# janinethoma/soft_contrastive_learning

Measured on AMD Instinct MI355X. Metric: train-step images/sec (VGG16-NetVLAD soft-MS, 640x480), higher is better.
Workload: dtype bf16; 1 GPU; configs[1]: wms soft-contrastive train step, VGG16-NetVLAD K=64, 24 images/GPU 640x480, bf16 backbone, float32-accurate NetVLAD + f32 loss; global_batch=24, locations=1200, parallelism=dp1, optimizer=adam

## Files before the change

### soft_contrastive_learning_amd/csrc/convh.hip

```cpp
#include <mutex>

#include "conv_lds.h"
#include "conv_pack_layout.h"

namespace {

constexpr int HBW = 40;
constexpr int HWC = HBW + 2;
constexpr int HPIX = 32;
constexpr int HCCH = 32;
constexpr int HNB = 128;
constexpr int HTPB = 3;
constexpr int HWT = 4 * HNB * 8;
constexpr int HTHR = 512;
constexpr int HX = 1;

template <int BHv>
struct HCfg {
  static constexpr int BH = BHv == 24 ? 12 : BHv;
  static constexpr int WR = BH + 2;
  static constexpr int SLOTS = WR * HWC * 4;
  static constexpr int NI = (SLOTS + 511) / 512;
  static constexpr int NA = (NI + 1) / 2;
  static constexpr int WIN = NI * 8 * 512;
  static constexpr int NMT = BH / 2 * 5;
  static constexpr int MT = BHv == 24 ? 15 : BH == 12 ? 8 : BH == 8 ? 10 : 4;
  static constexpr int NT = (BHv == 24 || BH == 8) ? 2 : 4;
  static constexpr int SPT = BHv == 24 ? 3 : 2;
  static constexpr int MH = MT / SPT;
  static constexpr size_t LDS = (2 * (size_t)WIN + 3 * HTPB * (size_t)HWT) * 2;
};

template <int V>
struct HConst {
  static constexpr int value = V;
};

__device__ __forceinline__ int ht_row(int i) { return (i >= 4 && i < 12) ? 1 : 0; }
__device__ __forceinline__ int ht_col(int i) { return i < 4 ? i : i < 8 ? i - 4 : i < 12 ? i - 4 : i - 8; }

__global__ __launch_bounds__(256) void convh_pack_kernel(const void* __restrict__ w, int64_t sk,
                                                         int64_t sc, int64_t sh, int64_t sw,
                                                         int flags, int cin, int kout,
                                                         unsigned short* __restrict__ packed) {
  const int transposed = flags & 1, wf32 = flags & 2;
  const int64_t idx = (int64_t)blockIdx.x * 256 + threadIdx.x;
  const int64_t total = (int64_t)9 * (cin / HCCH) * kout * HCCH;
  if (idx >= total) return;
  const int64_t off = pack_src_offset(pack_lds_coord(idx, cin), sk, sc, sh, sw, transposed);
  packed[idx] = weight_bf16(w, off, wf32);
}

template <int EPI, int BHv, bool STAMP = false, bool FULL = false>
__global__ __launch_bounds__(HTHR, 1) void convh_kernel(const unsigned short* __restrict__ x,
                                                       const unsigned short* __restrict__ packed,
                                                       int B, int H, int W, int cin, int kout,
                                                       unsigned short* __restrict__ out,
                                                       const float* __restrict__ bias, int relu,
                                                       const unsigned short* __restrict__ mask,
                                                       unsigned char* __restrict__ pidx,
                                                       int vblocks) {
  using G = HCfg<BHv>;
  constexpr int BH = G::BH, WR = G::WR, WIN = G::WIN, NMT = G::NMT, MT = G::MT, NT = G::NT;
  constexpr int MH = G::MH, NI = G::NI, NA = G::NA, SPT = G::SPT;
  constexpr bool WEAVE = BHv == 24 || BHv == 6 || BHv == 8;
  constexpr int HS = 9 * SPT;
  extern __shared__ __attribute__((aligned(16))) unsigned short lds[];
  unsigned short* win = lds;
  unsigned short* wts = lds + 2 * WIN;
  const int lane = threadIdx.x & 63;
  const int wid = __builtin_amdgcn_readfirstlane(threadIdx.x >> 6);
  const int i = lane & 15, g = lane >> 4;
  const int kb = kout / HNB;
  const int blocks_x = (W + HBW - 1) / HBW, blocks_y = (H + BH - 1) / BH;
  const int CC = cin / HCCH, S = 9 * CC;
  const unsigned short* zeros = reinterpret_cast<const unsigned short*>(zero_block);
  int nb = 0, b = 0, y0 = 0, x0 = 0;
  int rel[NI];
#pragma unroll
  for (int n = 0; n < NI; ++n) {
    const int slot = 64 * (wid + 8 * n) + lane;
    const int pix = slot >> 2, row = pix / HWC, col = pix - row * HWC;
    const int piece = (slot & 3) ^ (((col >> 2) & 1) | ((row & 1) << 1));
    rel[n] = pix >= WR * HWC ? -1 : (row << 16) | (col << 8) | piece;
  }
  int woff[NI];
  auto locate = [&](int vb) -> bool {
    const int grp = vb / (8 * kb), rem = vb - grp * 8 * kb;
    const int pblk = grp * 8 + (rem & 7);
    nb = rem >> 3;
    if (pblk >= B * blocks_x * blocks_y) return false;
    b = pblk / (blocks_x * blocks_y);
    const int t2 = pblk % (blocks_x * blocks_y);
    y0 = (t2 / blocks_x) * BH;
    x0 = (t2 % blocks_x) * HBW;
#pragma unroll
    for (int n = 0; n < NI; ++n) {
      int r = rel[n];
      asm volatile("" : "+v"(r));
      const int y = y0 - 1 + (r >> 16), xx = x0 - 1 + ((r >> 8) & 255);
      const bool inimg = r >= 0 && y >= 0 && y < H && xx >= 0 && xx < W;
      woff[n] = inimg ? ((b * H + y) * W + xx) * cin + 8 * (r & 255) : -1;
    }
    return true;
  };
  auto issue_win = [&](int cc, int buf, int n0, int n1) {
    const unsigned base = lds_byte_of(win) + buf * WIN * 2;
#pragma unroll
    for (int n = 0; n < NI; ++n)
      if (n >= n0 && n < n1)
        glds16(woff[n] >= 0 ? x + woff[n] + HCCH * cc : zeros, base + (wid + 8 * n) * 1024);
  };
  auto issue_wts = [&](int grp, int buf) {
    const unsigned short* src = packed + ((int64_t)nb * S + HTPB * grp) * HWT + lane * 8;
    const unsigned base = lds_byte_of(wts) + buf * HTPB * HWT * 2;
#pragma unroll
    for (int n = 0; n < 3; ++n) {
      const int j = wid + 8 * n;
      glds16(src + j * 512, base + j * 1024);
    }
  };
  auto issue_wts_one = [&](int grp, int buf, int n) {
    const unsigned short* src = packed + ((int64_t)nb * S + HTPB * grp) * HWT + lane * 8;
    const unsigned base = lds_byte_of(wts) + buf * HTPB * HWT * 2;
    const int j = wid + 8 * n;
    glds16(src + j * 512, base + j * 1024);
  };
  auto stage_first = [&]() {
    issue_wts(0, 0);
    issue_wts(1, 1);
    issue_win(0, 0, 0, NI);
  };
  const int mg = NT == 4 ? wid >> 1 : wid >> 2, ng = NT == 4 ? wid & 1 : wid & 3;
  constexpr bool REG = MT % 5 == 0;
  constexpr bool ALLT = NMT % MT == 0;
  int aoff[MT];
#pragma unroll
  for (int j = 0; j < MT; ++j) {
    const int mt = MT * mg + j < NMT ? MT * mg + j : NMT - 1;
    aoff[j] = ((2 * (mt / 5)) * HWC + 8 * (mt % 5)) * HPIX;
  }
  const int lane_a = (ht_row(i) * HWC + ht_col(i)) * HPIX + (REG ? 2 * (MT / 5) * mg * HWC * HPIX : 0);
  int pieces = 0;
#pragma unroll
  for (int t = 0; t < 9; ++t) {
    const int r = ht_row(i) + t / 3, c = ht_col(i) + t % 3;
    pieces |= (g ^ (((c >> 2) & 1) | ((r & 1) << 1))) << (2 * t);
  }
  const int lane_b = (g * HNB + 16 * NT * ng + i) * 8;

  const int relu_in = relu;
  const int dbg = STAMP ? 0 : SCL_DIAG_ONLY(relu >> 1);
  relu &= 1;
  const short relu_floor = relu ? (short)0 : (short)-32768;
  bool staged = false;
  if (!STAMP && (dbg & 4) && wid >= 4) __builtin_amdgcn_s_setprio(1);
  uint64_t stamp[STAMP ? 24 : 1];
  int tcount = 0;
#define HSTAMP(k)                                                                     \
  if (STAMP)                                                                          \
  asm volatile("s_memtime %0\n\ts_waitcnt lgkmcnt(0)" : "=s"(stamp[STAMP ? (k) : 0])::"memory")
  for (int vb = blockIdx.x; vb < vblocks; vb += gridDim.x) {
    HSTAMP(0);
    if (!staged) {
      if (!locate(vb)) continue;
      stage_first();
    }
    staged = false;
    const int nb_t = nb, b_t = b, y0_t = y0, x0_t = x0;

    f32x4 acc[MT][NT];
#pragma unroll
    for (int j = 0; j < MT; ++j)
#pragma unroll
      for (int n = 0; n < NT; ++n) acc[j][n] = f32x4{0.f, 0.f, 0.f, 0.f};

    u32x4 af[2][MH], bf[2][NT];
    int tb = 0;
    auto load_half = [&](const unsigned short* wbase, int h, int par, int apar) {
      const int t = h / SPT, mh = h % SPT;
      if (mh == 0) {
        const unsigned short* wbp = wts + t * HWT + lane_b;
#pragma unroll
        for (int n = 0; n < NT; ++n)
          bf[(t + par) & 1][n] = *reinterpret_cast<const u32x4*>(wbp + 16 * n * 8);
        int pk = pieces;
        asm volatile("" : "+v"(pk));
        tb = lane_a + ((pk >> (2 * t)) & 3) * 8;
      }
#pragma unroll
      for (int j = 0; j < MH; ++j)
        af[(h + apar) & 1][j] = *reinterpret_cast<const u32x4*>(
            wbase + tb +
            (REG ? (2 * ((MH * mh + j) / 5) * HWC + 8 * ((MH * mh + j) % 5)) * HPIX : aoff[MH * mh + j]) +
            ((t / 3) * HWC + t % 3) * HPIX);
    };
    const int NG = 3 * CC;
    auto chunk = [&](int cc, auto par_c) {
      constexpr int PAR = decltype(par_c)::value;
      constexpr int APAR = PAR * (HS & 1);
      const unsigned short* wcur = win + (cc & 1) * WIN;
      const unsigned short* wnext = win + ((cc + 1) & 1) * WIN;
      const int ccn = cc + 1 < CC ? cc + 1 : cc;
      auto issue_op = [&](int gi, int k) {
        if (k < 3) {
          const int gn = 3 * cc + gi + 2 < NG ? 3 * cc + gi + 2 : NG - 3 + (gi + 2) % 3;
          issue_wts_one(gn, (gi + 2) % 3, k);
        } else {
          const int n = (gi == 0 ? 0 : NA) + k - 3;
          if (gi == 0 && n < NA) issue_win(ccn, (cc + 1) & 1, n, n + 1);
          if (gi == 1 && n < NI) issue_win(ccn, (cc + 1) & 1, n, n + 1);
        }
      };
#pragma unroll
      for (int h = 0; h < HS; ++h) {
        if (h + 1 < HS)
          load_half(wcur, h + 1, PAR, APAR);
        else
          load_half(wnext, 0, PAR ^ 1, APAR ^ (HS & 1));
        __builtin_amdgcn_sched_barrier(0);
        const int t = h / SPT, mh = h % SPT;
        const bool after_barrier = WEAVE && (h % (3 * SPT) == HX + 1);
#pragma unroll
        for (int j = 0; j < MH; ++j) {
#pragma unroll
          for (int n = 0; n < NT; ++n)
            acc[MH * mh + j][n] =
                EPI == 3 ? mfma16b(af[(h + APAR) & 1][j], bf[(t + PAR) & 1][n], acc[MH * mh + j][n])
                         : mfma16b(bf[(t + PAR) & 1][n], af[(h + APAR) & 1][j], acc[MH * mh + j][n]);
          if (after_barrier) {
            __builtin_amdgcn_sched_barrier(0);
#pragma unroll
            for (int k = j * 6 / MH; k < (j + 1) * 6 / MH; ++k) issue_op(h / (3 * SPT), k);
            __builtin_amdgcn_sched_barrier(0);
          }
        }
        if (h % (3 * SPT) == HX) {
          __builtin_amdgcn_sched_barrier(0);
          const int gi = h / (3 * SPT);
          if (gi == 1)
            asm volatile("s_waitcnt vmcnt(%0)" ::"n"(NA) : "memory");
          else
            asm volatile("s_waitcnt vmcnt(0)" ::: "memory");
          HSTAMP(2 + 9 * PAR + 3 * gi);
          __builtin_amdgcn_s_barrier();
          HSTAMP(2 + 9 * PAR + 3 * gi + 1);
          if (!WEAVE) {
            const int gn = 3 * cc + gi + 2 < NG ? 3 * cc + gi + 2 : NG - 3 + (gi + 2) % 3;
            issue_wts(gn, (gi + 2) % 3);
            if (gi == 0) issue_win(ccn, (cc + 1) & 1, 0, NA);
            if (gi == 1) issue_win(ccn, (cc + 1) & 1, NA, NI);
          }
          HSTAMP(2 + 9 * PAR + 3 * gi + 2);
        }
      }
    };

    if (!(dbg & 1)) {
      asm volatile("s_waitcnt vmcnt(0)" ::: "memory");
      __syncthreads();
    }
    HSTAMP(1);
    load_half(win, 0, 0, 0);
#pragma unroll 1
    for (int cc = 0; cc < CC; cc += 2) {
      chunk(cc, HConst<0>());
      chunk(cc + 1, HConst<1>());
    }

    int nb_e = nb_t, b_e = b_t, y0_e = y0_t, x0_e = x0_t;
    asm volatile("" : "+s"(nb_e), "+s"(b_e), "+s"(y0_e), "+s"(x0_e));
    HSTAMP(20);
    __builtin_amdgcn_s_barrier();
    HSTAMP(21);
    constexpr int SLD = 16 * NT + 8;
    constexpr int PCS = 2 * NT;
    constexpr int RR = 16 * PCS / 64;
    constexpr int SCRW = 16 * SLD + 8 * (16 * NT + 16);
    static_assert(4 * SCRW <= WIN && 4 * SCRW <= HTPB * HWT, "epilogue scratch must fit");
    unsigned short* scr = wid < 4 ? lds + WIN + wid * SCRW : wts + 2 * HTPB * HWT + (wid - 4) * SCRW;
    const int ch_w = HNB * nb_e + 16 * NT * ng;
    f32x4 bias4[EPI == 1 ? NT : 1];
    float bias1[EPI == 3 ? NT : 1];
    if (EPI == 1) {
#pragma unroll
      for (int n = 0; n < NT; ++n)
        bias4[n] = *reinterpret_cast<const f32x4*>(bias + ch_w + 16 * n + 4 * g);
    }
    if (EPI == 3) {
#pragma unroll
      for (int n = 0; n < NT; ++n) bias1[n] = bias[ch_w + 16 * n + i];
    }
    int piece_o[RR], piece_px[RR];
#pragma unroll
    for (int rr = 0; rr < RR; ++rr) {
      const int pp = lane + 64 * rr;
      piece_px[rr] = pp / PCS;
      piece_o[rr] = (ht_row(pp / PCS) * W + ht_col(pp / PCS)) * kout + 8 * (pp % PCS);
    }
    constexpr int PD = MT / 2;
    u32x4 mk[EPI == 2 ? MT : 1][EPI == 2 ? RR : 1];
    const int64_t tile_off = (((int64_t)b_e * H + y0_e) * W + x0_e) * kout + ch_w;
    const bool full_tile = FULL ? !(dbg & 2) : (y0_e + BH <= H && x0_e + HBW <= W && !(dbg & 2));
    auto load_mask = [&](int j) {
      const int mt = MT * mg + j;
      const int oy = y0_e + 2 * (mt / 5), ox = x0_e + 8 * (mt % 5);
      const unsigned short* mb = mask + tile_off + ((2 * (mt / 5)) * W + 8 * (mt % 5)) * kout;
#pragma unroll
      for (int rr = 0; rr < RR; ++rr) {
        if (FULL ? (ALLT || mt < NMT) : (full_tile && mt < NMT)) {
          mk[EPI == 2 ? j : 0][EPI == 2 ? rr : 0] = *reinterpret_cast<const u32x4*>(mb + piece_o[rr]);
        } else if (FULL) {
          mk[EPI == 2 ? j : 0][EPI == 2 ? rr : 0] = u32x4{0u, 0u, 0u, 0u};
        } else {
          const bool inside = mt < NMT && oy + ht_row(piece_px[rr]) < H && ox + ht_col(piece_px[rr]) < W;
          mk[EPI == 2 ? j : 0][EPI == 2 ? rr : 0] =
              inside ? *reinterpret_cast<const u32x4*>(mb + piece_o[rr]) : u32x4{0u, 0u, 0u, 0u};
        }
      }
    };
    if (EPI == 2) {
#pragma unroll
      for (int j = 0; j < PD; ++j) load_mask(j);
    }

    auto stage_next = [&]() {
      const int vn = vb + gridDim.x;
      if (vn < vblocks && locate(vn)) {
        asm volatile("s_waitcnt vmcnt(0)" ::: "memory");
        stage_first();
        staged = true;
      }
    };
    if (EPI != 2) stage_next();

    if (EPI == 3) {
      const int PH = H / 2, PW = W / 2;
      const bool upper = g == 0 || g == 3;
      const int cb = g < 2 ? 0 : 4;
      unsigned char* scr8 = reinterpret_cast<unsigned char*>(scr + 16 * SLD);
      constexpr int SLD8 = 16 * NT + 16;
#pragma unroll
      for (int jb = 0; jb < MT; jb += 4) {
#pragma unroll
        for (int jj = 0; jj < 4; ++jj) {
          const int j = jb + jj < MT ? jb + jj : MT - 1;
#pragma unroll
          for (int n = 0; n < NT; ++n) {
#pragma unroll
            for (int q0 = 0; q0 < 4; q0 += 2) {
              const float v0 = acc[j][n][q0], v1 = acc[j][n][q0 + 1];
              const float lm = fmaxf(v0, v1);
              const int li = v0 >= v1 ? 0 : 1;
              const float om = __shfl_xor(lm, 16);
              const int oi = __shfl_xor(li, 16);
              const float mu = upper ? lm : om, ml = upper ? om : lm;
              const int iu = upper ? li : oi, il = upper ? oi : li;
              const float m = fmaxf(mu, ml);
              const int k = mu >= ml ? iu : 2 + il;
              const int pl = 4 * jj + ((cb + q0) >> 1);
              if (upper) {
                scr[pl * SLD + 16 * n + i] = f32_to_bf16(fmaxf(m + bias1[n], 0.f));
                scr8[pl * SLD8 + 16 * n + i] = (unsigned char)k;
              }
            }
          }
        }
        __builtin_amdgcn_wave_barrier();
#pragma unroll
        for (int rr = 0; rr < RR; ++rr) {
          const int pp = lane + 64 * rr, pl = pp / PCS, pc = pp % PCS;
          const int mt = MT * mg + jb + (pl >> 2);
          const int py = (y0_e >> 1) + mt / 5, px = (x0_e >> 1) + 4 * (mt % 5) + (pl & 3);
          const u32x4 v = *reinterpret_cast<const u32x4*>(scr + pl * SLD + 8 * pc);
          if (jb + (pl >> 2) < MT && (FULL ? (ALLT || mt < NMT) : (mt < NMT && py < PH && px < PW && !(dbg & 2))))
            *reinterpret_cast<u32x4*>(out + (((int64_t)b_e * PH + py) * PW + px) * kout + ch_w + 8 * pc) = v;
        }
        if (lane < 16 * NT) {
          const int pl = lane / NT, pc = lane % NT;
          const int mt = MT * mg + jb + (pl >> 2);
          const int py = (y0_e >> 1) + mt / 5, px = (x0_e >> 1) + 4 * (mt % 5) + (pl & 3);
          const u32x4 v = *reinterpret_cast<const u32x4*>(scr8 + pl * SLD8 + 16 * pc);
          if (jb + (pl >> 2) < MT && (FULL ? (ALLT || mt < NMT) : (mt < NMT && py < PH && px < PW && !(dbg & 2))))
            *reinterpret_cast<u32x4*>(pidx + (((int64_t)b_e * PH + py) * PW + px) * kout + ch_w + 16 * pc) = v;
        }
        __builtin_amdgcn_wave_barrier();
      }
    } else {
      unsigned short* out_tile = out + tile_off;
#pragma unroll
      for (int j = 0; j < MT; ++j) {
        const int mt = MT * mg + j;
        if (ALLT || mt < NMT) {
          const int oy = y0_e + 2 * (mt / 5), ox = x0_e + 8 * (mt % 5);
          unsigned short* ob = out_tile + ((2 * (mt / 5)) * W + 8 * (mt % 5)) * kout;
#pragma unroll
          for (int n = 0; n < NT; ++n) {
            f32x4 v = acc[j][n];
            if (EPI == 1) v += bias4[n];
            unsigned p0 = pack2_bf16(v[0], v[1]), p1 = pack2_bf16(v[2], v[3]);
            if (EPI == 1) {
              p0 = max2_i16(p0, relu_floor);
              p1 = max2_i16(p1, relu_floor);
            }
            const u32x2 pk = {p0, p1};
            *reinterpret_cast<u32x2*>(scr + i * SLD + 16 * n + 4 * g) = pk;
          }
          __builtin_amdgcn_wave_barrier();
#pragma unroll
          for (int rr = 0; rr < RR; ++rr) {
            u32x4 v = *reinterpret_cast<const u32x4*>(scr + piece_px[rr] * SLD + 8 * ((lane + 64 * rr) % PCS));
            if (EPI == 2) v = relu_mask(v, mk[EPI == 2 ? j : 0][EPI == 2 ? rr : 0]);
            if (full_tile) {
              *reinterpret_cast<u32x4*>(ob + piece_o[rr]) = v;
            } else if (!FULL) {
              const bool inside = oy + ht_row(piece_px[rr]) < H && ox + ht_col(piece_px[rr]) < W && !(dbg & 2);
              if (inside) *reinterpret_cast<u32x4*>(ob + piece_o[rr]) = v;
            }
          }
          __builtin_amdgcn_wave_barrier();
        }
        if (EPI == 2) {
          __builtin_amdgcn_sched_barrier(0);
          if (j + PD < MT) load_mask(j + PD);
          if (j + PD == MT - 1) stage_next();
          __builtin_amdgcn_sched_barrier(0);
        }
      }
    }
    if (STAMP) {
      HSTAMP(22);
      if (threadIdx.x == 64 * ((relu_in >> 4) & 7) && (tcount == 1 || tcount == 2)) {
        uint64_t* o = reinterpret_cast<uint64_t*>(out + (int64_t)B * H * W * kout) +
                      (int64_t)(blockIdx.x * 2 + tcount - 1) * 24;
#pragma unroll
        for (int k = 0; k < 23; ++k) o[k] = stamp[STAMP ? k : 0];
      }
      ++tcount;
    }
  }
#undef HSTAMP
}

}

struct HGeom {
  const unsigned short* packed;
  int bh;
  LdsConvGrid grid;
};

template <int E, int BHV, bool STAMP = false, bool FULL = false>
static void convh_run(const LdsConvCall& c, const HGeom& g, int relu) {
  if constexpr (!STAMP && !FULL)
    if (c.H % HCfg<BHV>::BH == 0 && c.W % HBW == 0) return convh_run<E, BHV, false, true>(c, g, relu);
  static SclDeviceOnce once;
  scl_call_once(once, [] {
    (void)hipFuncSetAttribute(reinterpret_cast<const void*>(&convh_kernel<E, BHV, STAMP, FULL>),
                              hipFuncAttributeMaxDynamicSharedMemorySize, (int)HCfg<BHV>::LDS);
  });
  SCL_LAUNCH("convh_kernel", (convh_kernel<E, BHV, STAMP, FULL>), dim3(g.grid.gsize), dim3(HTHR),
             HCfg<BHV>::LDS, c.stream, (const unsigned short*)c.x, g.packed, c.B, c.H, c.W, c.cin,
             c.kout, (unsigned short*)c.out, c.bias, relu, (const unsigned short*)c.mask,
             (unsigned char*)c.pidx, g.grid.vblocks);
}
template <int BHV>
static void convh_epilogue(const LdsConvCall& c, const HGeom& g, int dbgbits) {
  if (c.pidx) convh_run<3, BHV>(c, g, dbgbits);
  else if (c.mask) convh_run<2, BHV>(c, g, dbgbits);
  else if (c.bias) convh_run<1, BHV>(c, g, (c.relu ? 1 : 0) | dbgbits);
  else convh_run<0, BHV>(c, g, 0);
}

#ifdef SCL_DIAG
static bool convh_diag(const LdsConvCall& c, const HGeom& g, int* rc);
#endif

int convh_launch(const LdsConvCall& c) {
  const int dv = SCL_DIAG_ONLY(c.dv);
  HGeom g;
  g.packed = (const unsigned short*)c.workspace;
  if (c.flags & SCL_W_PACKED) {
    g.packed = (const unsigned short*)c.w;
  } else {
    const int64_t total = (int64_t)9 * (c.cin / HCCH) * c.kout * HCCH;
    SCL_LAUNCH("convh_pack_kernel", convh_pack_kernel, dim3((unsigned)((total + 255) / 256)),
               dim3(256), 0, c.stream, c.w, c.sk, c.sc, c.sh, c.sw, c.flags, c.cin, c.kout,
               (unsigned short*)c.workspace);
  }
  const int bx = (c.W + HBW - 1) / HBW, kb = c.kout / HNB;
  const int cus = scl_conv_cus();
  g.bh = 12;
  int64_t best = -1;
  for (int cand : {12, 8, 6}) {
    const int64_t wg = (int64_t)c.B * ((c.H + cand - 1) / cand) * bx * kb;
    const int64_t cost = ((wg + cus - 1) / cus) * (cand + 2);
    if (best < 0 || cost < best) {
      best = cost;
      g.bh = cand;
    }
  }
  if (dv == 3012 || dv == 3008 || dv == 3006) g.bh = dv - 3000;
  if (dv == 3013) g.bh = 12;
  g.grid = lds_conv_grid((int64_t)c.B * ((c.H + g.bh - 1) / g.bh) * bx, kb, cus, dv);
#ifdef SCL_DIAG
  {
    int rc;
    if (convh_diag(c, g, &rc)) return rc;
  }
#endif
  const int dbgbits = (dv >= 3020 && dv < 3024) ? (dv - 3020) << 1 : (dv == 3040 ? 4 << 1 : 0);
  if (g.bh == 12) convh_epilogue<24>(c, g, dbgbits);
  else if (g.bh == 8) convh_epilogue<8>(c, g, dbgbits);
  else convh_epilogue<6>(c, g, dbgbits);
  return scl_launch_status();
}
```

### soft_contrastive_learning_amd/csrc/scl_common.h

```cpp
#pragma once
#include <hip/hip_runtime.h>
#include <stdint.h>
#include <stdlib.h>
#include <atomic>
#include <mutex>
#include <type_traits>

#include "scl_hip.h"
#include "scl_cdna4.h"

#define SCL_WAVE 64

__device__ __forceinline__ f32x16 zero16() {
  f32x16 z;
#pragma unroll
  for (int i = 0; i < 16; ++i) z[i] = 0.f;
  return z;
}

__device__ __forceinline__ float bf16_to_f32(unsigned short v) {
  return __uint_as_float(((unsigned)v) << 16);
}
__device__ __forceinline__ unsigned short f32_to_bf16(float f) {
  __bf16 b = (__bf16)f;
  return __builtin_bit_cast(unsigned short, b);
}

__device__ __forceinline__ unsigned pack2_bf16(float a, float b) {
  typedef __bf16 bf16x2_t __attribute__((ext_vector_type(2)));
  typedef float f32x2_t __attribute__((ext_vector_type(2)));
  const f32x2_t v = {a, b};
  return __builtin_bit_cast(unsigned, __builtin_convertvector(v, bf16x2_t));
}

__device__ __forceinline__ unsigned max2_i16(unsigned w, short floor16) {
  typedef short s16x2_t __attribute__((ext_vector_type(2)));
  const s16x2_t a = __builtin_bit_cast(s16x2_t, w), z = {floor16, floor16};
  return __builtin_bit_cast(unsigned, __builtin_elementwise_max(a, z));
}

__device__ __forceinline__ unsigned short weight_bf16(const void* w, int64_t i, int f32) {
  return f32 ? f32_to_bf16(static_cast<const float*>(w)[i])
             : static_cast<const unsigned short*>(w)[i];
}
__device__ __forceinline__ void store_weight_grad(void* gw, int64_t i, float v, int f32) {
  if (f32)
    static_cast<float*>(gw)[i] = v;
  else
    static_cast<unsigned short*>(gw)[i] = f32_to_bf16(v);
}

__device__ __forceinline__ unsigned relu_mask_word(unsigned g, unsigned y) {
  unsigned keep, out;
  asm("v_pk_max_i16 %0, %1, 0" : "=v"(keep) : "v"(y));
  asm("v_pk_min_i16 %0, %1, 1 op_sel_hi:[1,0]" : "=v"(keep) : "v"(keep));
  asm("v_pk_mul_lo_u16 %0, %1, %2" : "=v"(out) : "v"(g), "v"(keep));
  return out;
}
template <typename V4>
__device__ __forceinline__ V4 relu_mask(V4 g, V4 y) {
  return V4{relu_mask_word(g.x, y.x), relu_mask_word(g.y, y.y), relu_mask_word(g.z, y.z),
               relu_mask_word(g.w, y.w)};
}

template <typename T>
struct Elem;
template <>
struct Elem<float> {
  static __device__ __forceinline__ float ld(const float* p) { return *p; }
  static __device__ __forceinline__ f32x4 ld4(const float* p) {
    return *reinterpret_cast<const f32x4*>(p);
  }
  static __device__ __forceinline__ f32x2 ld2(const float* p) {
    return *reinterpret_cast<const f32x2*>(p);
  }
  static __device__ __forceinline__ void st(float* p, float v) { *p = v; }
};
template <>
struct Elem<unsigned short> {
  static __device__ __forceinline__ float ld(const unsigned short* p) { return bf16_to_f32(*p); }
  static __device__ __forceinline__ f32x4 ld4(const unsigned short* p) {
    u16x4 v = *reinterpret_cast<const u16x4*>(p);
    f32x4 r;
    r[0] = bf16_to_f32(v[0]);
    r[1] = bf16_to_f32(v[1]);
    r[2] = bf16_to_f32(v[2]);
    r[3] = bf16_to_f32(v[3]);
    return r;
  }
  static __device__ __forceinline__ f32x2 ld2(const unsigned short* p) {
    const unsigned v = *reinterpret_cast<const unsigned*>(p);
    f32x2 r;
    r[0] = __uint_as_float(v << 16);
    r[1] = __uint_as_float(v & 0xffff0000u);
    return r;
  }
  static __device__ __forceinline__ void st(unsigned short* p, float v) { *p = f32_to_bf16(v); }
};

struct UnpoolFlags {
  unsigned e[2][4];
};
__device__ __forceinline__ UnpoolFlags unpool_flags(unsigned i0, unsigned i1) {
  UnpoolFlags f;
#pragma unroll
  for (int hw = 0; hw < 2; ++hw) {
    const unsigned iw = hw ? i1 : i0;
    const unsigned b0 = (iw << 7) & 0x80808080u, b1 = (iw << 6) & 0x80808080u;
    f.e[hw][3] = b0 & b1;
    f.e[hw][2] = b1 ^ f.e[hw][3];
    f.e[hw][1] = b0 ^ f.e[hw][3];
    f.e[hw][0] = (b0 | b1) ^ 0x80808080u;
  }
  return f;
}
template <typename V4>
__device__ __forceinline__ V4 unpool8(V4 g, const UnpoolFlags& f, int pos) {
  V4 o;
#pragma unroll
  for (int hw = 0; hw < 2; ++hw) {
    const unsigned e = f.e[hw][pos], eh = e << 8;
    o[2 * hw] = g[2 * hw] & __builtin_amdgcn_perm(eh, e, 0x08080a0au);
    o[2 * hw + 1] = g[2 * hw + 1] & __builtin_amdgcn_perm(eh, e, 0x09090b0bu);
  }
  return o;
}

template <typename T>
struct Raw;
template <>
struct Raw<float> {
  typedef f32x4 v4;
  typedef f32x2 v2;
  static __device__ __forceinline__ v4 ld4(const float* p) { return *reinterpret_cast<const v4*>(p); }
  static __device__ __forceinline__ v2 ld2(const float* p) { return *reinterpret_cast<const v2*>(p); }
  static __device__ __forceinline__ f32x4 cvt4(v4 r) { return r; }
  static __device__ __forceinline__ f32x2 cvt2(v2 r) { return r; }
  static __device__ __forceinline__ v4 ones4() { return v4{1.f, 1.f, 1.f, 1.f}; }
};
template <>
struct Raw<unsigned short> {
  typedef u16x4 v4;
  typedef unsigned v2;
  static __device__ __forceinline__ v4 ld4(const unsigned short* p) {
    return *reinterpret_cast<const v4*>(p);
  }
  static __device__ __forceinline__ v2 ld2(const unsigned short* p) {
    return *reinterpret_cast<const v2*>(p);
  }
  static __device__ __forceinline__ f32x4 cvt4(v4 r) {
    return f32x4{bf16_to_f32(r[0]), bf16_to_f32(r[1]), bf16_to_f32(r[2]), bf16_to_f32(r[3])};
  }
  static __device__ __forceinline__ f32x2 cvt2(v2 r) {
    return f32x2{__uint_as_float(r << 16), __uint_as_float(r & 0xffff0000u)};
  }
  static __device__ __forceinline__ v4 ones4() { return v4{0x3f80, 0x3f80, 0x3f80, 0x3f80}; }
};

__device__ __forceinline__ float half_sum(float v) {
#pragma unroll
  for (int m = 1; m < 32; m <<= 1) v += __shfl_xor(v, m, 64);
  return v;
}
__device__ __forceinline__ float half_max(float v) {
#pragma unroll
  for (int m = 1; m < 32; m <<= 1) v = fmaxf(v, __shfl_xor(v, m, 64));
  return v;
}
__device__ __forceinline__ float wave_sum(float v) {
#pragma unroll
  for (int m = 1; m < 64; m <<= 1) v += __shfl_xor(v, m, 64);
  return v;
}
__device__ __forceinline__ float wave_max(float v) {
#pragma unroll
  for (int m = 1; m < 64; m <<= 1) v = fmaxf(v, __shfl_xor(v, m, 64));
  return v;
}
__device__ __forceinline__ float wave_min(float v) {
#pragma unroll
  for (int m = 1; m < 64; m <<= 1) v = fminf(v, __shfl_xor(v, m, 64));
  return v;
}

template <int OP>
__device__ __forceinline__ float block_reduce(float v, float* scratch) {
  const int lane = threadIdx.x & 63, wid = threadIdx.x >> 6, nw = (blockDim.x + 63) >> 6;
  v = OP == 0 ? wave_sum(v) : (OP == 1 ? wave_max(v) : wave_min(v));
  __syncthreads();
  if (lane == 0) scratch[wid] = v;
  __syncthreads();
  float r = scratch[0];
  for (int i = 1; i < nw; ++i) {
    float o = scratch[i];
    r = OP == 0 ? r + o : (OP == 1 ? fmaxf(r, o) : fminf(r, o));
  }
  return r;
}

struct SclProfSink {
  int capacity;
  int count;
  hipEvent_t* ev;
  const char** name;
};
extern SclProfSink* volatile scl_prof_sink;

#define SCL_LAUNCH(kname, kernel, grid, block, lds, st, ...)                     \
  do {                                                                           \
    SclProfSink* ps_ = scl_prof_sink;                                            \
    int slot_ = -1;                                                              \
    if (ps_) {                                                                   \
      slot_ = __atomic_fetch_add(&ps_->count, 1, __ATOMIC_RELAXED);              \
      if (slot_ >= ps_->capacity) slot_ = -1;                                    \
    }                                                                            \
    if (slot_ >= 0) {                                                            \
      ps_->name[slot_] = (kname);                                                \
      (void)hipEventRecord(ps_->ev[2 * slot_], (st));                            \
    }                                                                            \
    hipLaunchKernelGGL(kernel, grid, block, lds, (st), __VA_ARGS__);             \
    if (slot_ >= 0) (void)hipEventRecord(ps_->ev[2 * slot_ + 1], (st));          \
  } while (0)

#ifdef SCL_DIAG
extern volatile int scl_debug_variant;
static inline int scl_variant() { return scl_debug_variant; }
#define SCL_DIAG_ONLY(x) (x)
#else
static constexpr int scl_variant() { return 0; }
#define SCL_DIAG_ONLY(x) 0
#endif

extern volatile int scl_reserve_cus;
static inline int scl_usable_cus(int cus) {
  int reserve = scl_reserve_cus;
  if (reserve < 0) {
    const char* e = getenv("SCL_RESERVE_CUS");
    reserve = e ? atoi(e) : 0;
    if (reserve < 0) reserve = 0;
    scl_reserve_cus = reserve;
  }
  const int left = cus - reserve;
  return left >= 8 ? left : (cus < 8 ? cus : 8);
}

static inline int scl_device_cus() {
  static std::atomic<int> table[64];
  int dev = 0;
  if (hipGetDevice(&dev) != hipSuccess || dev < 0 || dev >= 64) return 256;
  int n = table[dev].load(std::memory_order_relaxed);
  if (n == 0) {
    int c = 0;
    n = (hipDeviceGetAttribute(&c, hipDeviceAttributeMultiprocessorCount, dev) == hipSuccess && c > 0) ? c : 256;
    table[dev].store(n, std::memory_order_relaxed);
  }
  return n;
}

constexpr int kSclMaxConvCus = 1024;
static inline int scl_conv_cus() {
  const int u = scl_usable_cus(scl_device_cus());
  return u > kSclMaxConvCus ? kSclMaxConvCus : u;
}

struct SclDeviceOnce { std::once_flag f[64]; };
template <class F> static inline void scl_call_once(SclDeviceOnce& o, F&& fn) {
  int d = 0;
  if (hipGetDevice(&d) != hipSuccess || d < 0 || d >= 64) d = 0;
  std::call_once(o.f[d], fn);
}
template <auto Kernel> static inline void scl_lds_limit(int bytes) {
  static SclDeviceOnce once;
  scl_call_once(once, [bytes] {
    (void)hipFuncSetAttribute(reinterpret_cast<const void*>(Kernel),
                              hipFuncAttributeMaxDynamicSharedMemorySize, bytes);
  });
}

static inline int scl_launch_status() { return (int)hipGetLastError(); }
static inline bool scl_aligned256(const void* p) { return (((uintptr_t)p) & 255u) == 0; }
static inline size_t scl_round256(size_t n) { return (n + 255u) & ~(size_t)255u; }

struct Carver {
  char* base;
  size_t off = 0;
  explicit Carver(void* p) : base((char*)p) {}
  template <class T> T* take(size_t count) {
    T* ptr = (T*)(base + off);
    off += scl_round256(count * sizeof(T));
    return ptr;
  }
  float* take(size_t floats) { return take<float>(floats); }
};
```

Before: 2038 images/sec.

## Prefetch ReLU-backward mask into packed keep bits during conv main loop

For the EPI==2 (ReLU-backward masked) full-tile BHv=24 conv path, the mask loads now happen inside the main K loop. One dwordx4 is issued per weight group and packed into 16-bit keep bitfields held in four registers, so the epilogue applies the mask from registers instead of loading it there. The per-slot rel[] table is dropped and window offsets are recomputed from mbcnt lane ids, and the epilogue also re-derives its lane id. This is meant to lower register pressure and hide mask load latency, at the cost of extra VALU work, vmcnt waits interleaved with weight loads, and more complex code.

```diff
diff --git a/soft_contrastive_learning_amd/csrc/convh.hip b/soft_contrastive_learning_amd/csrc/convh.hip
--- a/soft_contrastive_learning_amd/csrc/convh.hip
+++ b/soft_contrastive_learning_amd/csrc/convh.hip
@@ -36,6 +36,12 @@
   static constexpr int value = V;
 };
 
+__device__ __forceinline__ int lane_now() {
+  int l;
+  asm volatile("v_mbcnt_lo_u32_b32 %0, -1, 0\n\tv_mbcnt_hi_u32_b32 %0, -1, %0" : "=v"(l));
+  return l;
+}
+
 __device__ __forceinline__ int ht_row(int i) { return (i >= 4 && i < 12) ? 1 : 0; }
 __device__ __forceinline__ int ht_col(int i) { return i < 4 ? i : i < 8 ? i - 4 : i < 12 ? i - 4 : i - 8; }
 
@@ -65,6 +71,12 @@
   constexpr int MH = G::MH, NI = G::NI, NA = G::NA, SPT = G::SPT;
   constexpr bool WEAVE = BHv == 24 || BHv == 6 || BHv == 8;
   constexpr int HS = 9 * SPT;
+  constexpr int PCS = 2 * NT;
+  constexpr int RR = 16 * PCS / 64;
+  constexpr int NP = MT * RR;
+  constexpr bool AHEAD = EPI == 2 && BHv == 24 && FULL;
+  static_assert(NP <= 16, "a tile's keep bits fill four registers");
+  static_assert(!AHEAD || (MT % 5 == 0 && NMT % MT == 0 && RR == 1), "AHEAD: whole row pairs, one piece per m-tile");
   extern __shared__ __attribute__((aligned(16))) unsigned short lds[];
   unsigned short* win = lds;
   unsigned short* wts = lds + 2 * WIN;
@@ -76,14 +88,6 @@
   const int CC = cin / HCCH, S = 9 * CC;
   const unsigned short* zeros = reinterpret_cast<const unsigned short*>(zero_block);
   int nb = 0, b = 0, y0 = 0, x0 = 0;
-  int rel[NI];
-#pragma unroll
-  for (int n = 0; n < NI; ++n) {
-    const int slot = 64 * (wid + 8 * n) + lane;
-    const int pix = slot >> 2, row = pix / HWC, col = pix - row * HWC;
-    const int piece = (slot & 3) ^ (((col >> 2) & 1) | ((row & 1) << 1));
-    rel[n] = pix >= WR * HWC ? -1 : (row << 16) | (col << 8) | piece;
-  }
   int woff[NI];
   auto locate = [&](int vb) -> bool {
     const int grp = vb / (8 * kb), rem = vb - grp * 8 * kb;
@@ -94,13 +98,15 @@
     const int t2 = pblk % (blocks_x * blocks_y);
     y0 = (t2 / blocks_x) * BH;
     x0 = (t2 % blocks_x) * HBW;
+    const int l = lane_now();
 #pragma unroll
     for (int n = 0; n < NI; ++n) {
-      int r = rel[n];
-      asm volatile("" : "+v"(r));
-      const int y = y0 - 1 + (r >> 16), xx = x0 - 1 + ((r >> 8) & 255);
-      const bool inimg = r >= 0 && y >= 0 && y < H && xx >= 0 && xx < W;
-      woff[n] = inimg ? ((b * H + y) * W + xx) * cin + 8 * (r & 255) : -1;
+      const int slot = 64 * (wid + 8 * n) + l;
+      const int pix = slot >> 2, row = pix / HWC, col = pix - row * HWC;
+      const int piece = (slot & 3) ^ (((col >> 2) & 1) | ((row & 1) << 1));
+      const int y = y0 - 1 + row, xx = x0 - 1 + col;
+      const bool inimg = pix < WR * HWC && y >= 0 && y < H && xx >= 0 && xx < W;
+      woff[n] = inimg ? ((b * H + y) * W + xx) * cin + 8 * piece : -1;
     }
     return true;
   };
@@ -157,6 +163,7 @@
   if (!STAMP && (dbg & 4) && wid >= 4) __builtin_amdgcn_s_setprio(1);
   uint64_t stamp[STAMP ? 24 : 1];
   int tcount = 0;
+  u32x4 mfly = {0u, 0u, 0u, 0u};
 #define HSTAMP(k)                                                                     \
   if (STAMP)                                                                          \
   asm volatile("s_memtime %0\n\ts_waitcnt lgkmcnt(0)" : "=s"(stamp[STAMP ? (k) : 0])::"memory")
@@ -194,6 +201,35 @@
             wbase + tb +
             (REG ? (2 * ((MH * mh + j) / 5) * HWC + 8 * ((MH * mh + j) % 5)) * HPIX : aoff[MH * mh + j]) +
             ((t / 3) * HWC + t % 3) * HPIX);
+    };
+    unsigned mbits[4] = {0u, 0u, 0u, 0u};
+    const unsigned short* mask_w = mask;
+    unsigned mlane = 0u;
+    if (AHEAD) {
+      mask_w = mask + ((((int64_t)b_t * H + y0_t + 2 * (MT / 5) * mg) * W + x0_t) * kout + HNB * nb_t + 16 * NT * ng);
+      const int l = lane_now();
+      mlane = 2u * ((ht_row(l / PCS) * W + ht_col(l / PCS)) * kout + 8 * (l % PCS));
+    }
+    auto mask_issue = [&](int q) {
+      const int r2 = q / 5, c5 = q - 5 * r2;
+      const bool live = q < NP;
+      const unsigned short* base = live ? mask_w + (int64_t)((2 * r2 * W + 8 * c5) * kout) : zeros;
+      const unsigned off = live ? mlane : 0u;
+      asm volatile("global_load_dwordx4 %0, %1, %2" : "=v"(mfly) : "v"(off), "s"(base) : "memory");
+    };
+    auto mask_convert = [&](int q) {
+      u32x4 m = mfly;
+      asm volatile("" : "+v"(m));
+      unsigned a = relu_keep_word(m.x);
+      a |= relu_keep_word(m.y) << 2;
+      a |= relu_keep_word(m.z) << 4;
+      a |= relu_keep_word(m.w) << 6;
+      a <<= (q & 1) + 4 * (q & 2);
+#pragma unroll
+      for (int r = 0; r < 4; ++r) mbits[r] |= a & ((q >> 2) == r ? ~0u : 0u);
+    };
+    auto mask_keep = [&](int q, int d) -> unsigned {
+      return (mbits[q >> 2] >> ((q & 1) + 4 * (q & 2) + 2 * d)) & 0x00010001u;
     };
     const int NG = 3 * CC;
     auto chunk = [&](int cc, auto par_c) {
@@ -242,6 +278,10 @@
             asm volatile("s_waitcnt vmcnt(%0)" ::"n"(NA) : "memory");
           else
             asm volatile("s_waitcnt vmcnt(0)" ::: "memory");
+          if (AHEAD && 3 * cc + gi <= NP) {
+            mask_convert(3 * cc + gi - 1);
+            mask_issue(3 * cc + gi);
+          }
           HSTAMP(2 + 9 * PAR + 3 * gi);
           __builtin_amdgcn_s_barrier();
           HSTAMP(2 + 9 * PAR + 3 * gi + 1);
@@ -268,14 +308,27 @@
       chunk(cc + 1, HConst<1>());
     }
 
+    if (AHEAD) {
+      asm volatile("s_waitcnt vmcnt(0)" ::: "memory");
+      if (NG <= NP) {
+        mask_convert(NG - 1);
+#pragma unroll 1
+        for (int q = NG; q < NP; ++q) {
+          mask_issue(q);
+          asm volatile("s_waitcnt vmcnt(0)" ::: "memory");
+          mask_convert(q);
+        }
+      }
+      asm volatile("" ::"v"(mfly));
+    }
     int nb_e = nb_t, b_e = b_t, y0_e = y0_t, x0_e = x0_t;
     asm volatile("" : "+s"(nb_e), "+s"(b_e), "+s"(y0_e), "+s"(x0_e));
+    const int lane_e = ((EPI == 3 && BHv == 24) || !FULL || AHEAD) ? lane_now() : lane;
+    const int i_e = lane_e & 15, g_e = lane_e >> 4;
     HSTAMP(20);
     __builtin_amdgcn_s_barrier();
     HSTAMP(21);
     constexpr int SLD = 16 * NT + 8;
-    constexpr int PCS = 2 * NT;
-    constexpr int RR = 16 * PCS / 64;
     constexpr int SCRW = 16 * SLD + 8 * (16 * NT + 16);
     static_assert(4 * SCRW <= WIN && 4 * SCRW <= HTPB * HWT, "epilogue scratch must fit");
     unsigned short* scr = wid < 4 ? lds + WIN + wid * SCRW : wts + 2 * HTPB * HWT + (wid - 4) * SCRW;
@@ -285,21 +338,22 @@
     if (EPI == 1) {
 #pragma unroll
       for (int n = 0; n < NT; ++n)
-        bias4[n] = *reinterpret_cast<const f32x4*>(bias + ch_w + 16 * n + 4 * g);
+        bias4[n] = *reinterpret_cast<const f32x4*>(bias + ch_w + 16 * n + 4 * g_e);
     }
     if (EPI == 3) {
 #pragma unroll
-      for (int n = 0; n < NT; ++n) bias1[n] = bias[ch_w + 16 * n + i];
+      for (int n = 0; n < NT; ++n) bias1[n] = bias[ch_w + 16 * n + i_e];
     }
     int piece_o[RR], piece_px[RR];
 #pragma unroll
     for (int rr = 0; rr < RR; ++rr) {
-      const int pp = lane + 64 * rr;
+      const int pp = lane_e + 64 * rr;
       piece_px[rr] = pp / PCS;
       piece_o[rr] = (ht_row(pp / PCS) * W + ht_col(pp / PCS)) * kout + 8 * (pp % PCS);
     }
+    constexpr bool MASK_EPI = EPI == 2 && !AHEAD;
     constexpr int PD = MT / 2;
-    u32x4 mk[EPI == 2 ? MT : 1][EPI == 2 ? RR : 1];
+    u32x4 mk[MASK_EPI ? MT : 1][MASK_EPI ? RR : 1];
     const int64_t tile_off = (((int64_t)b_e * H + y0_e) * W + x0_e) * kout + ch_w;
     const bool full_tile = FULL ? !(dbg & 2) : (y0_e + BH <= H && x0_e + HBW <= W && !(dbg & 2));
     auto load_mask = [&](int j) {
@@ -309,17 +363,17 @@
 #pragma unroll
       for (int rr = 0; rr < RR; ++rr) {
         if (FULL ? (ALLT || mt < NMT) : (full_tile && mt < NMT)) {
-          mk[EPI == 2 ? j : 0][EPI == 2 ? rr : 0] = *reinterpret_cast<const u32x4*>(mb + piece_o[rr]);
+          mk[MASK_EPI ? j : 0][MASK_EPI ? rr : 0] = *reinterpret_cast<const u32x4*>(mb + piece_o[rr]);
         } else if (FULL) {
-          mk[EPI == 2 ? j : 0][EPI == 2 ? rr : 0] = u32x4{0u, 0u, 0u, 0u};
+          mk[MASK_EPI ? j : 0][MASK_EPI ? rr : 0] = u32x4{0u, 0u, 0u, 0u};
         } else {
           const bool inside = mt < NMT && oy + ht_row(piece_px[rr]) < H && ox + ht_col(piece_px[rr]) < W;
-          mk[EPI == 2 ? j : 0][EPI == 2 ? rr : 0] =
+          mk[MASK_EPI ? j : 0][MASK_EPI ? rr : 0] =
               inside ? *reinterpret_cast<const u32x4*>(mb + piece_o[rr]) : u32x4{0u, 0u, 0u, 0u};
         }
       }
     };
-    if (EPI == 2) {
+    if (MASK_EPI) {
 #pragma unroll
       for (int j = 0; j < PD; ++j) load_mask(j);
     }
@@ -332,12 +386,12 @@
         staged = true;
       }
     };
-    if (EPI != 2) stage_next();
+    if (!MASK_EPI) stage_next();
 
     if (EPI == 3) {
       const int PH = H / 2, PW = W / 2;
-      const bool upper = g == 0 || g == 3;
-      const int cb = g < 2 ? 0 : 4;
+      const bool upper = g_e == 0 || g_e == 3;
+      const int cb = g_e < 2 ? 0 : 4;
       unsigned char* scr8 = reinterpret_cast<unsigned char*>(scr + 16 * SLD);
       constexpr int SLD8 = 16 * NT + 16;
 #pragma unroll
@@ -360,8 +414,8 @@
               const int k = mu >= ml ? iu : 2 + il;
               const int pl = 4 * jj + ((cb + q0) >> 1);
               if (upper) {
-                scr[pl * SLD + 16 * n + i] = f32_to_bf16(fmaxf(m + bias1[n], 0.f));
-                scr8[pl * SLD8 + 16 * n + i] = (unsigned char)k;
+                scr[pl * SLD + 16 * n + i_e] = f32_to_bf16(fmaxf(m + bias1[n], 0.f));
+                scr8[pl * SLD8 + 16 * n + i_e] = (unsigned char)k;
               }
             }
           }
@@ -369,15 +423,15 @@
         __builtin_amdgcn_wave_barrier();
 #pragma unroll
         for (int rr = 0; rr < RR; ++rr) {
-          const int pp = lane + 64 * rr, pl = pp / PCS, pc = pp % PCS;
+          const int pp = lane_e + 64 * rr, pl = pp / PCS, pc = pp % PCS;
           const int mt = MT * mg + jb + (pl >> 2);
           const int py = (y0_e >> 1) + mt / 5, px = (x0_e >> 1) + 4 * (mt % 5) + (pl & 3);
           const u32x4 v = *reinterpret_cast<const u32x4*>(scr + pl * SLD + 8 * pc);
           if (jb + (pl >> 2) < MT && (FULL ? (ALLT || mt < NMT) : (mt < NMT && py < PH && px < PW && !(dbg & 2))))
             *reinterpret_cast<u32x4*>(out + (((int64_t)b_e * PH + py) * PW + px) * kout + ch_w + 8 * pc) = v;
         }
-        if (lane < 16 * NT) {
-          const int pl = lane / NT, pc = lane % NT;
+        if (lane_e < 16 * NT) {
+          const int pl = lane_e / NT, pc = lane_e % NT;
           const int mt = MT * mg + jb + (pl >> 2);
           const int py = (y0_e >> 1) + mt / 5, px = (x0_e >> 1) + 4 * (mt % 5) + (pl & 3);
           const u32x4 v = *reinterpret_cast<const u32x4*>(scr8 + pl * SLD8 + 16 * pc);
@@ -404,13 +458,18 @@
               p1 = max2_i16(p1, relu_floor);
             }
             const u32x2 pk = {p0, p1};
-            *reinterpret_cast<u32x2*>(scr + i * SLD + 16 * n + 4 * g) = pk;
+            *reinterpret_cast<u32x2*>(scr + i_e * SLD + 16 * n + 4 * g_e) = pk;
           }
           __builtin_amdgcn_wave_barrier();
 #pragma unroll
           for (int rr = 0; rr < RR; ++rr) {
-            u32x4 v = *reinterpret_cast<const u32x4*>(scr + piece_px[rr] * SLD + 8 * ((lane + 64 * rr) % PCS));
-            if (EPI == 2) v = relu_mask(v, mk[EPI == 2 ? j : 0][EPI == 2 ? rr : 0]);
+            u32x4 v = *reinterpret_cast<const u32x4*>(scr + piece_px[rr] * SLD + 8 * ((lane_e + 64 * rr) % PCS));
+            if (MASK_EPI) v = relu_mask(v, mk[MASK_EPI ? j : 0][MASK_EPI ? rr : 0]);
+            if (AHEAD) {
+              const int q = j * RR + rr;
+              v = u32x4{relu_apply_word(v.x, mask_keep(q, 0)), relu_apply_word(v.y, mask_keep(q, 1)),
+                        relu_apply_word(v.z, mask_keep(q, 2)), relu_apply_word(v.w, mask_keep(q, 3))};
+            }
             if (full_tile) {
               *reinterpret_cast<u32x4*>(ob + piece_o[rr]) = v;
             } else if (!FULL) {
@@ -420,7 +479,7 @@
           }
           __builtin_amdgcn_wave_barrier();
         }
-        if (EPI == 2) {
+        if (MASK_EPI) {
           __builtin_amdgcn_sched_barrier(0);
           if (j + PD < MT) load_mask(j + PD);
           if (j + PD == MT - 1) stage_next();
diff --git a/soft_contrastive_learning_amd/csrc/scl_common.h b/soft_contrastive_learning_amd/csrc/scl_common.h
--- a/soft_contrastive_learning_amd/csrc/scl_common.h
+++ b/soft_contrastive_learning_amd/csrc/scl_common.h
@@ -50,12 +50,19 @@
     static_cast<unsigned short*>(gw)[i] = f32_to_bf16(v);
 }
 
-__device__ __forceinline__ unsigned relu_mask_word(unsigned g, unsigned y) {
-  unsigned keep, out;
+__device__ __forceinline__ unsigned relu_keep_word(unsigned y) {
+  unsigned keep;
   asm("v_pk_max_i16 %0, %1, 0" : "=v"(keep) : "v"(y));
   asm("v_pk_min_i16 %0, %1, 1 op_sel_hi:[1,0]" : "=v"(keep) : "v"(keep));
+  return keep;
+}
+__device__ __forceinline__ unsigned relu_apply_word(unsigned g, unsigned keep) {
+  unsigned out;
   asm("v_pk_mul_lo_u16 %0, %1, %2" : "=v"(out) : "v"(g), "v"(keep));
   return out;
+}
+__device__ __forceinline__ unsigned relu_mask_word(unsigned g, unsigned y) {
+  return relu_apply_word(g, relu_keep_word(y));
 }
 template <typename V4>
 __device__ __forceinline__ V4 relu_mask(V4 g, V4 y) {
```

Result: no change. 2053 images/sec (median of 6 runs) (+0.7%).
